# pfe-rs/lk-s-2022-estimacija-pokreta

Hardware: AMD Instinct MI355X
Metric: Mpix/s flow (1024x436, bcd_times=4) (higher is better)
Workload: dtype f64; 1 GPU; single 1024x436 Sintel-shape pair per step per GPU, forward only, bcd_times=4 (BASELINE.json configs[1]); cells 64x27, 150 labels/px; pairs_in_flight_per_gpu=7, mode=batch

## Files before the change

lk-s-2022-estimacija-pokreta_amd/csrc/bcd.hip:

```cpp
#include "dflow_common.h"

#define BCD_THREADS 192
#ifndef BCD_MINWAVES
#define BCD_MINWAVES 5
#endif
#define BCD_MASK_WORDS 5
#define BCD_BLK 5
#define BCD_LIST 15
#define BCD_LDS_LABELS 256
#define BCD_TB_STEPS 32
#define BCD_GROUPS 3
#define BCD_CAP_B01 40
#define BCD_CAP_B2 16
#define BCD_CAP_C01 24
#define BCD_CAP_C2 8
#define BCD_ROW_B (2 * BCD_CAP_B01 + BCD_CAP_B2)
#define BCD_ROW_C (2 * BCD_CAP_C01 + BCD_CAP_C2)
#define BCD_ROW_BC (BCD_ROW_B + BCD_ROW_C + 2)
#define BCD_POOL_DIV 32

#define BLK_MORE 0x800u
#define BLK_HAS_B 0x8000u
#define BLK_HAS_C 0x80000u
#define BLK_EMPTY_X 0xFFFFFFFFu
#define BLK_EMPTY_Y 0x000000FFu

__device__ static inline void chain_geom(int phase, int chain, int H, int W, int &ty, int &tx, int &ys, int &xs, int &len)
{
    if (phase == 0) { ty = 0; tx = 2 * chain; ys = 1; xs = 0; len = H; }
    else if (phase == 1) { ty = 2 * chain; tx = W - 1; ys = 0; xs = -1; len = W; }
    else if (phase == 2) { ty = H - 1; tx = (W / 2) * 2 - 1 - 2 * chain; ys = -1; xs = 0; len = H; }
    else { ty = (H / 2) * 2 - 1 - 2 * chain; tx = 0; ys = 0; xs = 1; len = W; }
}

struct BcdPlanes {
    uint8_t *back;
    uint2 *lab;
    uint2 *blkA;
    uint2 *blkBC;
    uint32_t *masks;
    uint32_t *cursor;
    uint32_t pool_rows;
};

#ifndef BCD_RANGE_BYTES
#define BCD_RANGE_BYTES 768
#endif
#define BCD_RANGE_R (BCD_RANGE_BYTES - 1)
#ifndef BCD_RANGE_PITCH
#define BCD_RANGE_PITCH 5
#endif
#define BCD_RANGE_ENTRIES (DFLOW_MAX_LABELS + 1)
#ifndef BCD_LISTS_WAVE_LDS
#define BCD_LISTS_WAVE_LDS 4096
#endif
static_assert(BCD_RANGE_BYTES % 256 == 0 && BCD_RANGE_BYTES >= 256 && BCD_RANGE_BYTES <= 1024, "rank table: 1..4 dwords per lane");
static_assert(BCD_RANGE_BYTES + BCD_RANGE_ENTRIES * BCD_RANGE_PITCH * 4 <= BCD_LISTS_WAVE_LDS && BCD_LISTS_WAVE_LDS >= 1024, "a wave's LDS");
static_assert(BCD_RANGE_PITCH >= BCD_MASK_WORDS && BCD_RANGE_PITCH <= 8, "prefix-set entry pitch");

__device__ static inline void wave_lds_sync()
{
    __builtin_amdgcn_fence(__ATOMIC_RELEASE, "wavefront");
    __builtin_amdgcn_wave_barrier();
    __builtin_amdgcn_fence(__ATOMIC_ACQUIRE, "wavefront");
}
template <int CTRL, int ROWS = 0xF> __device__ static inline uint32_t dpp_or0(uint32_t v)
{
    return (uint32_t)__builtin_amdgcn_update_dpp(0, (int)v, CTRL, ROWS, 0xF, false);
}
__device__ static inline uint32_t wave_scan_add(uint32_t x)
{
    x += dpp_or0<0x111>(x); x += dpp_or0<0x112>(x); x += dpp_or0<0x114>(x); x += dpp_or0<0x118>(x);
    x += dpp_or0<0x142, 0xA>(x); x += dpp_or0<0x143, 0xC>(x);
    return x;
}
template <int CTRL, int ROWS = 0xF> __device__ static inline void sets_or_step(uint32_t (&x)[BCD_MASK_WORDS])
{
#pragma unroll
    for (int w = 0; w < BCD_MASK_WORDS; w++) x[w] |= dpp_or0<CTRL, ROWS>(x[w]);
}
__device__ static inline void wave_scan_or(uint32_t (&x)[BCD_MASK_WORDS])
{
    sets_or_step<0x111>(x); sets_or_step<0x112>(x); sets_or_step<0x114>(x); sets_or_step<0x118>(x);
    sets_or_step<0x142, 0xA>(x); sets_or_step<0x143, 0xC>(x);
}
template <int CTRL, int ROWS = 0xF> __device__ static inline int dpp_min(int v)
{
    return min(v, __builtin_amdgcn_update_dpp(v, v, CTRL, ROWS, 0xF, false));
}
__device__ static inline int wave_min(int x)
{
    x = dpp_min<0x111>(x); x = dpp_min<0x112>(x); x = dpp_min<0x114>(x); x = dpp_min<0x118>(x);
    x = dpp_min<0x142, 0xA>(x); x = dpp_min<0x143, 0xC>(x);
    return __builtin_amdgcn_readlane(x, 63);
}
__device__ static inline void sets_load(const uint32_t *e, uint32_t (&w)[BCD_MASK_WORDS])
{
    if constexpr (BCD_RANGE_PITCH % 4 == 0) {
        const uint4 a = *reinterpret_cast<const uint4 *>(e);
        w[0] = a.x; w[1] = a.y; w[2] = a.z; w[3] = a.w;
    } else if constexpr (BCD_RANGE_PITCH % 2 == 0) {
        const uint2 a = *reinterpret_cast<const uint2 *>(e), b = *reinterpret_cast<const uint2 *>(e + 2);
        w[0] = a.x; w[1] = a.y; w[2] = b.x; w[3] = b.y;
    } else {
        w[0] = e[0]; w[1] = e[1]; w[2] = e[2]; w[3] = e[3];
    }
    w[4] = e[4];
}
__device__ static inline void sets_store(uint32_t *e, const uint32_t (&w)[BCD_MASK_WORDS])
{
    if constexpr (BCD_RANGE_PITCH % 4 == 0) {
        *reinterpret_cast<uint4 *>(e) = make_uint4(w[0], w[1], w[2], w[3]);
    } else if constexpr (BCD_RANGE_PITCH % 2 == 0) {
        *reinterpret_cast<uint2 *>(e) = make_uint2(w[0], w[1]); *reinterpret_cast<uint2 *>(e + 2) = make_uint2(w[2], w[3]);
    } else {
        e[0] = w[0]; e[1] = w[1]; e[2] = w[2]; e[3] = w[3];
    }
    e[4] = w[4];
}
template <int AX> __device__ static inline int range_coord(uint32_t f)
{
    const int lo = (int)(f & 0xFFFFu), hi = (int)(f >> 16);
    return AX ? lo - hi + 65535 : lo + hi;
}

#ifndef BCD_LISTS_WAVES
#define BCD_LISTS_WAVES 8
#endif
__global__ void __launch_bounds__(256, BCD_LISTS_WAVES) bcd_lists_kernel(int H, int W, int LP, int tpsi, const uint32_t *__restrict__ proposals,
                                                        const float *__restrict__ lcosts, const int32_t *__restrict__ nprop,
                                                        BcdPlanes pl)
{
    __shared__ uint32_t s_cols[4][256];
    __shared__ __attribute__((aligned(16))) uint8_t s_wave[4][BCD_LISTS_WAVE_LDS];
    const int lane = threadIdx.x & 63, wv = threadIdx.x >> 6;
    const int q = (int)blockIdx.x * 4 + __builtin_amdgcn_readfirstlane(wv);
    if (q >= H * W) return;
    const int y = q / W, x = q % W;
    const int py = (x & 1) ? y + 1 : y - 1, sy = (x & 1) ? y - 1 : y + 1;
    const int px = (y & 1) ? x - 1 : x + 1, sx = (y & 1) ? x + 1 : x - 1;
    const bool start0 = py < 0 || py >= H, start1 = px < 0 || px >= W;
    const bool v0 = sy >= 0 && sy < H, v1 = sx >= 0 && sx < W;
    const int p0 = v0 ? sy * W + x : q, p1 = v1 ? y * W + sx : q;
    const int pn = nprop[q], tn0 = v0 ? nprop[p0] : 0, tn1 = v1 ? nprop[p1] : 0;
    const int half = lane >> 5;
    uint32_t fq[3], f[5];
#pragma unroll
    for (int j = 0; j < 3; j++) {
        const int k = lane + 64 * j;
        fq[j] = k < pn ? flow_bias(proposals[(size_t)q * LP + k]) : 0u;
        s_cols[wv][k] = fq[j];
    }
    s_cols[wv][192 + lane] = 0u;
#pragma unroll
    for (int j = 0; j < 2; j++) {
        const int k = lane + 64 * j;
        f[j] = k < tn0 ? flow_bias(proposals[(size_t)p0 * LP + k]) : 0u;
        f[2 + j] = k < tn1 ? flow_bias(proposals[(size_t)p1 * LP + k]) : 0u;
    }
    {
        const int k = 128 + (lane & 31);
        f[4] = k < (half ? tn1 : tn0) ? flow_bias(proposals[(size_t)(half ? p1 : p0) * LP + k]) : 0u;
    }
#pragma unroll
    for (int j = 0; j < 3; j++) {
        const int k = lane + 64 * j;
        if (k < LP) pl.lab[(size_t)q * LP + k] = make_uint2(fq[j], __float_as_uint(k < pn ? lcosts[(size_t)q * LP + k] : DFLOW_FILL_COST));
    }
    if (start0 || start1) {
#pragma unroll
        for (int j = 0; j < 3; j++) {
            const int k = lane + 64 * j;
            if (k < LP) {
                if (start0) pl.blkA[((size_t)q * 2 + 0) * LP + k] = make_uint2(BLK_EMPTY_X, BLK_EMPTY_Y);
                if (start1) pl.blkA[((size_t)q * 2 + 1) * LP + k] = make_uint2(BLK_EMPTY_X, BLK_EMPTY_Y);
            }
        }
    }
    if (!v0 && !v1) return;
    const uint32_t kbias = 0x80000000u - (uint32_t)tpsi;
    const uint32_t *__restrict__ colp = proposals + (size_t)q * LP;
    uint32_t m[5][BCD_MASK_WORDS];
    const bool fifth = LP > 128 && (tn0 > 128 || tn1 > 128);
    auto build = [&](auto with5) {
#pragma unroll
        for (int j = 0; j < BCD_MASK_WORDS; j++) {
#pragma unroll
            for (int g = 0; g < 5; g++) m[g][j] = 0xFFFFFFFFu;
            if (32 * j < pn) {
                const int nv = pn - 32 * j;
                auto cols8 = [&](auto hic) {
#pragma unroll
                    for (int cc = decltype(hic)::value; cc > decltype(hic)::value - 8; cc--) {
                        const uint32_t col = flow_bias(colp[32 * j + cc]);
#pragma unroll
                        for (int g = 0; g < 4; g++) m[g][j] = __builtin_amdgcn_alignbit(m[g][j], __builtin_amdgcn_sad_u16(col, f[g], kbias), 31);
                        if (decltype(with5)::value) m[4][j] = __builtin_amdgcn_alignbit(m[4][j], __builtin_amdgcn_sad_u16(col, f[4], kbias), 31);
                    }
                };
                if (nv > 24) cols8(IntC<31>());
                if (nv > 16) cols8(IntC<23>());
                if (nv > 8) cols8(IntC<15>());
                cols8(IntC<7>());
                if (nv < 32 && (nv & 7) != 0) {
                    const uint32_t inval = ~0u << nv;
#pragma unroll
                    for (int g = 0; g < 5; g++) m[g][j] |= inval;
                }
            }
        }
    };
    const int pt = min(pn, DFLOW_MAX_LABELS);
    int cq[2][3], org[2];
    bool wide = false;
#pragma unroll
    for (int j = 0; j < 3; j++) { cq[0][j] = range_coord<0>(fq[j]); cq[1][j] = range_coord<1>(fq[j]); }
#pragma unroll
    for (int ax = 0; ax < 2; ax++) {
        int mn = 1 << 18;
#pragma unroll
        for (int j = 0; j < 3; j++) if (lane + 64 * j < pt) mn = min(mn, cq[ax][j]);
        org[ax] = wave_min(mn);
#pragma unroll
        for (int j = 0; j < 3; j++) { cq[ax][j] -= org[ax]; wide |= lane + 64 * j < pt && cq[ax][j] >= BCD_RANGE_R; }
    }
    if (__ballot(wide)) {
        if (fifth) build(IntC<1>()); else build(IntC<0>());
    } else {
        constexpr int NW = BCD_RANGE_BYTES / 256;
        uint32_t *const cw = reinterpret_cast<uint32_t *>(&s_wave[wv][0]);
        const uint8_t *const cb = &s_wave[wv][0];
        uint32_t *const sets = reinterpret_cast<uint32_t *>(&s_wave[wv][BCD_RANGE_BYTES]);
        auto axis = [&](auto axc) {
            constexpr int AX = decltype(axc)::value;
#pragma unroll
            for (int i = 0; i < NW; i++) cw[lane * NW + i] = 0u;
            wave_lds_sync();
            uint32_t ord[3];
#pragma unroll
            for (int j = 0; j < 3; j++) {
                ord[j] = 0u;
                if (lane + 64 * j < pt) {
                    const uint32_t rel = (uint32_t)cq[AX][j], sh = 8u * (rel & 3u);
                    ord[j] = (atomicAdd(&cw[rel >> 2], 1u << sh) >> sh) & 0xFFu;
                }
            }
            wave_lds_sync();
            uint32_t t[NW], before[NW], tot = 0u;
#pragma unroll
            for (int i = 0; i < NW; i++) {
                t[i] = cw[lane * NW + i];
                t[i] += t[i] << 8; t[i] += t[i] << 16;
                before[i] = tot; tot += t[i] >> 24;
            }
            const uint32_t lower = wave_scan_add(tot) - tot;
#pragma unroll
            for (int i = 0; i < NW; i++) {
                const uint32_t base = lower + before[i];
                cw[lane * NW + i] = (t[i] << 8) + __builtin_amdgcn_perm(base, base, 0x00000000u);
            }
            if (lane == 0) {
                const uint32_t none[BCD_MASK_WORDS] = {0u, 0u, 0u, 0u, 0u};
                sets_store(sets, none);
            }
            wave_lds_sync();
#pragma unroll
            for (int j = 0; j < 3; j++) {
                if (lane + 64 * j < pt) {
                    const uint32_t r = (uint32_t)cb[cq[AX][j]] + ord[j], bit = 1u << (lane & 31);
                    uint32_t one[BCD_MASK_WORDS] = {0u, 0u, 0u, 0u, 0u};
                    one[2 * j] = half ? 0u : bit;
                    if (j < 2) one[2 * j + 1] = half ? bit : 0u;
                    sets_store(sets + (r + 1u) * BCD_RANGE_PITCH, one);
                }
            }
            wave_lds_sync();
            uint32_t a[3][BCD_MASK_WORDS];
#pragma unroll
            for (int i = 0; i < 3; i++) {
#pragma unroll
                for (int w = 0; w < BCD_MASK_WORDS; w++) a[i][w] = 0u;
                if (3 * lane + i <= pt) sets_load(sets + (3 * lane + i) * BCD_RANGE_PITCH, a[i]);
            }
#pragma unroll
            for (int w = 0; w < BCD_MASK_WORDS; w++) { a[1][w] |= a[0][w]; a[2][w] |= a[1][w]; }
            wave_scan_or(a[2]);
#pragma unroll
            for (int w = 0; w < BCD_MASK_WORDS; w++) {
                const uint32_t lower_lanes = dpp_or0<0x138>(a[2][w]);
                a[0][w] |= lower_lanes; a[1][w] |= lower_lanes;
            }
#pragma unroll
            for (int i = 0; i < 3; i++)
                if (3 * lane + i <= pt) sets_store(sets + (3 * lane + i) * BCD_RANGE_PITCH, a[i]);
            wave_lds_sync();
#pragma unroll
            for (int g = 0; g < 5; g++) {
                if (g < 4 || fifth) {
                    const int c = range_coord<AX>(f[g]) - org[AX];
                    const int hi = min(max(c + tpsi, 0), BCD_RANGE_R), lo = min(max(c - tpsi + 1, 0), BCD_RANGE_R);
                    uint32_t in[BCD_MASK_WORDS], out[BCD_MASK_WORDS];
                    sets_load(sets + (uint32_t)cb[hi] * BCD_RANGE_PITCH, in);
                    sets_load(sets + (uint32_t)cb[lo] * BCD_RANGE_PITCH, out);
#pragma unroll
                    for (int w = 0; w < BCD_MASK_WORDS; w++) {
                        if (AX == 0) m[g][w] = in[w] & ~out[w];
                        else m[g][w] = ~(m[g][w] & in[w] & ~out[w]);
                        asm("" : "+v"(m[g][w]));
                    }
                } else {
#pragma unroll
                    for (int w = 0; w < BCD_MASK_WORDS; w++) m[g][w] = 0xFFFFFFFFu;
                }
                if (g & 1) __builtin_amdgcn_sched_barrier(0);
            }
            wave_lds_sync();
        };
        axis(IntC<0>());
        axis(IntC<1>());
    }

    auto emit = [&](auto mergedc, const uint32_t (&mg)[BCD_MASK_WORDS], const uint32_t me, const int ig, const int tl, const int tn,
                    const bool valid, const size_t pd) {
        constexpr bool MERGED = decltype(mergedc)::value != 0;
        uint32_t w[BCD_MASK_WORDS];
        int cnt = 0;
        uint32_t dead = valid && tl < tn ? 0u : ~0u;
        asm("" : "+v"(dead));
#pragma unroll
        for (int j = 0; j < BCD_MASK_WORDS; j++) { w[j] = __builtin_amdgcn_bitop3_b32(mg[j], dead, 0u, 0x03); cnt += __popc(w[j]); }
        uint8_t *row = &s_wave[wv][16 * lane];
        *reinterpret_cast<uint4 *>(row) = make_uint4(0xFFFFFFFFu, 0xFFFFFFFFu, 0xFFFFFFFFu, 0xFFFFFFFFu);
        const int n = min(cnt, BCD_LIST);
        const bool any = __ballot(cnt > 0) != 0ull;
        if (any) {
            uint32_t wt[BCD_MASK_WORDS];
#pragma unroll
            for (int j = 0; j < BCD_MASK_WORDS; j++) wt[j] = w[j];
            if (__ballot(cnt > BCD_LIST)) {
                int extra = cnt - BCD_LIST;
#pragma unroll
                for (int j = BCD_MASK_WORDS - 1; j >= 0; j--)
                    while (extra > 0 && wt[j]) { wt[j] &= ~(0x80000000u >> __clz(wt[j])); extra--; }
            }
            uint8_t *ap = row;
#pragma unroll
            for (int j = 0; j < BCD_MASK_WORDS; j++) {
                uint32_t ww = wt[j];
                while (ww) { *ap++ = (uint8_t)(32 * j + __ffs(ww) - 1); ww &= ww - 1; }
            }
        }
        const uint4 lst = *reinterpret_cast<const uint4 *>(row);
        const uint32_t l0 = lst.x, l1 = lst.y, l2 = lst.z, l3 = lst.w;
        uint32_t c0 = 0u, c1 = 0u;
        if (any) {
            auto slots = [&](auto lo, auto hi) {
#pragma unroll
                for (int e = decltype(lo)::value; e < decltype(hi)::value; e++) {
                    const uint32_t word = e < 4 ? l0 : (e < 8 ? l1 : (e < 12 ? l2 : l3));
                    const uint32_t k = (word >> (8 * (e & 3))) & 0xFFu;
                    const uint32_t psi = flow_l1_biased(me, s_cols[wv][k]);
                    if (e < 8) c0 |= psi << (4 * e); else c1 |= psi << (4 * (e - 8));
                }
            };
            slots(IntC<0>(), IntC<BCD_BLK>());
            if (__ballot(n > BCD_BLK)) {
                slots(IntC<BCD_BLK>(), IntC<2 * BCD_BLK>());
                if (__ballot(n > 2 * BCD_BLK)) slots(IntC<2 * BCD_BLK>(), IntC<BCD_LIST>());
            }
        }
        const unsigned long long pp = (((unsigned long long)c1 << 32) | c0) & ~(~0ull << (4 * n));
        const unsigned long long hasB = __ballot(cnt > BCD_BLK), hasC = __ballot(cnt > 2 * BCD_BLK);
        uint32_t rankB = __builtin_amdgcn_mbcnt_hi((uint32_t)(hasB >> 32), __builtin_amdgcn_mbcnt_lo((uint32_t)hasB, 0u));
        uint32_t rankC = __builtin_amdgcn_mbcnt_hi((uint32_t)(hasC >> 32), __builtin_amdgcn_mbcnt_lo((uint32_t)hasC, 0u));
        if (MERGED && half) { rankB -= (uint32_t)__popc((uint32_t)hasB); rankC -= (uint32_t)__popc((uint32_t)hasC); }
        const uint32_t capB = ig < 2 ? BCD_CAP_B01 : BCD_CAP_B2, capC = ig < 2 ? BCD_CAP_C01 : BCD_CAP_C2;
        const bool storeB = cnt > BCD_BLK && rankB < capB, storeC = cnt > 2 * BCD_BLK && storeB && rankC < capC;
        const bool more = cnt > BCD_LIST || (cnt > BCD_BLK && !storeB) || (cnt > 2 * BCD_BLK && !storeC);
        const uint32_t ax = l0;
        const uint32_t ay = (l1 & 0xFFu) | (((uint32_t)pp & 0xFFFFFu) << 8) | (more ? BLK_MORE : 0u) | (storeB ? BLK_HAS_B : 0u) |
                            (storeC ? BLK_HAS_C : 0u) | ((uint32_t)(more ? 15 : min(cnt, 15)) << 28);
        const uint32_t bx = __builtin_amdgcn_alignbit(l2, l1, 8);
        const uint32_t by = ((l2 >> 8) & 0xFFu) | (((uint32_t)(pp >> 20) & 0xFFFFFu) << 8);
        const uint32_t cx = __builtin_amdgcn_alignbit(l3, l2, 16);
        const uint32_t cy = ((l3 >> 16) & 0xFFu) | (((uint32_t)(pp >> 40) & 0xFFFFFu) << 8);
        if (valid && tl < LP) pl.blkA[pd * (size_t)LP + tl] = make_uint2(ax, ay);
        if (storeB) pl.blkBC[pd * BCD_ROW_BC + ig * BCD_CAP_B01 + rankB] = make_uint2(bx, by);
        if (storeC) pl.blkBC[pd * BCD_ROW_BC + BCD_ROW_B + ig * BCD_CAP_C01 + rankC] = make_uint2(cx, cy);
        const unsigned long long dense = __ballot(more);
        if (dense) {
            uint32_t base = 0u;
            if (lane == 0) base = atomicAdd(pl.cursor, (uint32_t)__popcll(dense));
            base = (uint32_t)__builtin_amdgcn_readfirstlane((int)base);
            uint32_t rank = __builtin_amdgcn_mbcnt_hi((uint32_t)(dense >> 32), __builtin_amdgcn_mbcnt_lo((uint32_t)dense, 0u));
            if (MERGED) {
                const uint32_t nlo = (uint32_t)__popc((uint32_t)dense);
                if ((lane & 31) == 0 && (half ? (dense >> 32) != 0ull : (uint32_t)dense != 0u))
                    reinterpret_cast<uint32_t *>(pl.blkBC + pd * BCD_ROW_BC + BCD_ROW_B + BCD_ROW_C)[ig] = base + (half ? nlo : 0u);
            } else if (lane == 0) {
                reinterpret_cast<uint32_t *>(pl.blkBC + pd * BCD_ROW_BC + BCD_ROW_B + BCD_ROW_C)[ig] = base;
            }
            const uint32_t slot = base + rank;
            if (more && slot < pl.pool_rows) {
                uint32_t *out = pl.masks + (size_t)slot * BCD_MASK_WORDS;
#pragma unroll
                for (int j = 0; j < BCD_MASK_WORDS; j++) out[j] = w[j];
            }
        }
    };
    const size_t pd0 = (size_t)p0 * 2 + 0, pd1 = (size_t)p1 * 2 + 1;
    if (v0) {
        emit(IntC<0>(), m[0], f[0], 0, lane, tn0, true, pd0);
        if (LP > 64) emit(IntC<0>(), m[1], f[1], 1, 64 + lane, tn0, true, pd0);
    }
    if (v1) {
        emit(IntC<0>(), m[2], f[2], 0, lane, tn1, true, pd1);
        if (LP > 64) emit(IntC<0>(), m[3], f[3], 1, 64 + lane, tn1, true, pd1);
    }
    if (LP > 128) emit(IntC<1>(), m[4], f[4], 2, 128 + (lane & 31), half ? tn1 : tn0, half ? v1 : v0, half ? pd1 : pd0);
}

#ifndef BCD_MAX_BATCH
#define BCD_MAX_BATCH 8
#endif
struct BcdPass {
    const int32_t *nprop;
    int32_t *bestlabels;
    BcdPlanes pl;
};
struct BcdArgs {
    int H, W, LP, tpsi, phase;
    double lamda;
    BcdPass pass[BCD_MAX_BATCH];
};

struct Cand {
    double v; int k;
};

__device__ static inline void cand_min(Cand &a, double ov, int ok)
{
    const bool take = ov < a.v || (ov == a.v && ok < a.k);
    a.v = take ? ov : a.v;
    a.k = take ? ok : a.k;
}

template <int CTRL> __device__ static inline void cand_dpp(const Cand &a, double &ov, int &ok)
{
    const int lo = __double2loint(a.v), hi = __double2hiint(a.v);
    const int olo = __builtin_amdgcn_update_dpp(lo, lo, CTRL, 0xF, 0xF, false);
    const int ohi = __builtin_amdgcn_update_dpp(hi, hi, CTRL, 0xF, 0xF, false);
    ok = __builtin_amdgcn_update_dpp(a.k, a.k, CTRL, 0xF, 0xF, false);
    ov = __hiloint2double(ohi, olo);
}

#define DPP_ROW_SHL1 0x101
#define DPP_ROW_SHL2 0x102
#define DPP_ROW_SHL4 0x104
#define DPP_ROW_SHL8 0x108

__device__ static inline void wave_min_lane0(Cand &pm)
{
    double ov; int ok;
    cand_dpp<DPP_ROW_SHL1>(pm, ov, ok); cand_min(pm, ov, ok);
    cand_dpp<DPP_ROW_SHL2>(pm, ov, ok); cand_min(pm, ov, ok);
    cand_dpp<DPP_ROW_SHL4>(pm, ov, ok); cand_min(pm, ov, ok);
    cand_dpp<DPP_ROW_SHL8>(pm, ov, ok); cand_min(pm, ov, ok);
    const int lo = __double2loint(pm.v), hi = __double2hiint(pm.v);
#pragma unroll
    for (int r = 1; r < 4; r++) {
        const double rv = __hiloint2double(__builtin_amdgcn_readlane(hi, 16 * r), __builtin_amdgcn_readlane(lo, 16 * r));
        const int rk = __builtin_amdgcn_readlane(pm.k, 16 * r);
        cand_min(pm, rv, rk);
    }
}

__device__ static inline uint32_t wave_u32_min_asm(uint32_t x)
{
    asm volatile("s_nop 1\n\t"
                 "v_min_u32_dpp %0, %0, %0 row_shl:1 row_mask:0xf bank_mask:0xf\n\t"
                 "s_nop 1\n\t"
                 "v_min_u32_dpp %0, %0, %0 row_shl:2 row_mask:0xf bank_mask:0xf\n\t"
                 "s_nop 1\n\t"
                 "v_min_u32_dpp %0, %0, %0 row_shl:4 row_mask:0xf bank_mask:0xf\n\t"
                 "s_nop 1\n\t"
                 "v_min_u32_dpp %0, %0, %0 row_shl:8 row_mask:0xf bank_mask:0xf\n\t"
                 "s_nop 0"
                 : "+v"(x));
    const uint32_t a = (uint32_t)__builtin_amdgcn_readlane((int)x, 0), b = (uint32_t)__builtin_amdgcn_readlane((int)x, 16);
    const uint32_t c = (uint32_t)__builtin_amdgcn_readlane((int)x, 32), d = (uint32_t)__builtin_amdgcn_readlane((int)x, 48);
    const uint32_t ab = a < b ? a : b, cd = c < d ? c : d;
    return ab < cd ? ab : cd;
}
__device__ static inline unsigned long long wave_key_min_asm(unsigned long long key, int *first_lane)
{
    const uint32_t hi = (uint32_t)(key >> 32), lo = (uint32_t)key;
    const uint32_t mh = wave_u32_min_asm(hi);
    const unsigned long long tie = __ballot(hi == mh);
    uint32_t ml; int fl;
    fl = __ffsll((long long)tie) - 1;
    ml = (uint32_t)__builtin_amdgcn_readlane((int)lo, fl);
    if (__builtin_expect(__popcll(tie) != 1, 0)) {
        ml = wave_u32_min_asm(hi == mh ? lo : 0xFFFFFFFFu);
        fl = __ffsll((long long)__ballot(hi == mh && lo == ml)) - 1;
    }
    *first_lane = fl;
    return ((unsigned long long)mh << 32) | ml;
}

__device__ static inline uint32_t lane_rank(unsigned long long mask)
{
    return __builtin_amdgcn_mbcnt_hi((uint32_t)(mask >> 32), __builtin_amdgcn_mbcnt_lo((uint32_t)mask, 0u));
}

#define BCD_BACK_PITCH BCD_THREADS

typedef const __attribute__((address_space(1))) char *gptr_t;
__device__ static inline gptr_t uniform_ptr(const void *p)
{
    const unsigned long long v = (unsigned long long)p;
    const uint32_t lo = __builtin_amdgcn_readfirstlane((uint32_t)v), hi = __builtin_amdgcn_readfirstlane((uint32_t)(v >> 32));
    return (gptr_t)(((unsigned long long)hi << 32) | lo);
}
__device__ static inline unsigned long long ballot64(bool b) { return __builtin_amdgcn_ballot_w64(b); }

__global__ void __launch_bounds__(BCD_THREADS, BCD_MINWAVES) bcd_chain_kernel(BcdArgs a)
{
    __shared__ double s_dp[2 * BCD_LDS_LABELS];
    __shared__ unsigned long long permv[2 * 4];
    __shared__ int permi[2 * 4 + 4];
    __shared__ __attribute__((aligned(16))) uint8_t tb[BCD_TB_STEPS * BCD_BACK_PITCH];
    extern __shared__ __attribute__((aligned(16))) uint32_t s_dyn[];
    uint32_t *bestf = s_dyn + 1;
    int *tnl;
    int *s_label = permi + 8;

    const int tid = threadIdx.x, lane = tid & 63, wave = __builtin_amdgcn_readfirstlane(tid >> 6);
    const int chain = blockIdx.x;
    const int W = a.W, LP = a.LP;
    const bool owner = tid < LP;
    const unsigned long long ownmask = ballot64(owner);
    const int tl = owner ? tid : LP - 1;
    int ty0, tx0, ys, xs, len;
    chain_geom(a.phase, chain, a.H, W, ty0, tx0, ys, xs, len);
    const int pstep = ys * W + xs;
    const int pix0 = ty0 * W + tx0;
    const int dir = ys != 0 ? 0 : 1;
    const int dirp = ys + xs;
    const uint32_t tpsi = (uint32_t)a.tpsi;
    const double tpsi_d = (double)a.tpsi;
    const double lamda = a.lamda;
    const BcdPass &ps = a.pass[blockIdx.y];
    const int32_t *g_nprop = ps.nprop;
    int32_t *g_best = ps.bestlabels;
    const uint2 *g_lab = ps.pl.lab;
    const uint32_t *g_masks = ps.pl.masks;
    const uint2 *g_bc = ps.pl.blkBC;
    const uint32_t pool_rows = ps.pl.pool_rows;
    uint8_t *back = ps.pl.back + ((size_t)chain * len) * BCD_BACK_PITCH;

    tnl = (int *)(bestf + len + 2);
    for (int i = tid; i < 2 * BCD_LDS_LABELS; i += BCD_THREADS) s_dp[i] = 1e300;
    for (int i = tid; i < len; i += BCD_THREADS) {
        int pix = pix0 + i * pstep;
        bestf[i] = g_lab[(size_t)pix * LP + g_best[pix]].x;
        tnl[i] = g_nprop[pix];
    }
    if (tid == 0) { bestf[-1] = 0u; bestf[len] = 0u; bestf[len + 1] = 0u; }
    __syncthreads();

    const uint32_t offl = (uint32_t)tl * 8u;
    const long long rowl = (long long)LP * 8, rowg = (long long)BCD_ROW_BC * 8;
    const long long strA = (long long)pstep * 2 * rowl, strL = (long long)pstep * rowl, strG = (long long)pstep * 2 * rowg;
    gptr_t pA = uniform_ptr((const char *)ps.pl.blkA + ((long long)pix0 * 2 + dir) * rowl);
    gptr_t pL = uniform_ptr((const char *)ps.pl.lab + (long long)pix0 * rowl);
    gptr_t pB = uniform_ptr((const char *)ps.pl.blkBC + ((long long)pix0 * 2 + dir) * rowg + (long long)wave * (BCD_CAP_B01 * 8));
    const uint32_t coff = (uint32_t)(BCD_ROW_B * 8 + wave * (BCD_CAP_C01 * 8) - wave * (BCD_CAP_B01 * 8));
    int nextA = 0, nextG = 0;
    auto advA = [&]() { const bool m = nextA + 1 < len; pA += m ? strA : 0; pL += m ? strL : 0; nextA++; };
    auto advG = [&]() { const bool m = nextG + 1 < len; pB += m ? strG : 0; nextG++; };
    auto ld8 = [](gptr_t base, uint32_t off) {
        const unsigned long long v = *reinterpret_cast<const __attribute__((address_space(1))) unsigned long long *>(base + off);
        return make_uint2((uint32_t)v, (uint32_t)(v >> 32));
    };
    auto fetchBC = [&](const uint2 &blkA, uint2 &B, uint2 &C) {
        const bool hb = owner && (blkA.y & BLK_HAS_B) != 0u, hc = owner && (blkA.y & BLK_HAS_C) != 0u;
        const unsigned long long mb = ballot64(hb);
        B = make_uint2(BLK_EMPTY_X, BLK_EMPTY_Y); C = make_uint2(BLK_EMPTY_X, BLK_EMPTY_Y);
        if (mb) {
            if (hb) B = ld8(pB, lane_rank(mb) * 8u);
            const unsigned long long mc = ballot64(hc);
            if (mc) { if (hc) C = ld8(pB, coff + lane_rank(mc) * 8u); }
        }
        advG();
    };
    uint2 A0, L0 = ld8(pL, offl); advA();
    uint2 A1 = ld8(pA, offl), L1 = ld8(pL, offl); advA();
    uint2 A2 = ld8(pA, offl), L2 = ld8(pL, offl); advA();
    uint2 A3 = ld8(pA, offl), L3 = ld8(pL, offl); advA();
    uint2 B1, C1, B0, C0;
    advG();
    fetchBC(A1, B1, C1);
    fetchBC(A2, B0, C0);

    {
        const uint32_t Fc = L0.x;
        const int ip = dirp, im = -dirp;
        const uint32_t s1 = (ip >= 0 && ip < len) ? min(tpsi, flow_l1_biased(Fc, bestf[ip])) : 0u;
        const uint32_t s2 = (im >= 0 && im < len) ? min(tpsi, flow_l1_biased(Fc, bestf[im])) : 0u;
        unsigned long long key = ~0ull;
        if (owner && tl < tnl[0]) {
            const double d0 = __dadd_rn((double)(s1 + s2), __dmul_rn(lamda, (double)__uint_as_float(L0.y)));
            s_dp[tl] = d0;
            key = (unsigned long long)__double_as_longlong(__dadd_rn(tpsi_d, d0));
        }
        int fl;
        const unsigned long long m = wave_key_min_asm(key, &fl);
        if (lane == 0) { permv[wave] = m; permi[wave] = wave * 64 + fl; }
    }
    A0 = ld8(pA, offl); L0 = ld8(pL, offl); advA();
    __syncthreads();

    int pn = tnl[0];
    __attribute__((address_space(1))) uint8_t *backrow = (__attribute__((address_space(1))) uint8_t *)uniform_ptr(back + BCD_BACK_PITCH);
    int tn_nx = tnl[1];
    uint32_t bfp_nx = bestf[1 + dirp], bfm_nx = bestf[1 - dirp];
    auto step = [&](auto curc, auto edgec, const int i, uint2 &inA, uint2 &inL, uint2 &inB, uint2 &inC, const uint2 &nxA) __attribute__((always_inline)) {
        constexpr int CUR = decltype(curc)::value;
        constexpr bool EDGE = decltype(edgec)::value != 0;
        const char *prev = reinterpret_cast<const char *>(s_dp + (CUR ^ 1) * BCD_LDS_LABELS);
        const int tn = tn_nx;
        const uint32_t bfp = bfp_nx, bfm = bfm_nx;
        tn_nx = tnl[min(i + 1, len - 1)];
        bfp_nx = bestf[i + 1 + dirp]; bfm_nx = bestf[i + 1 - dirp];
        const uint32_t ax = inA.x, ay = inA.y, bx = inB.x, by = inB.y, cx = inC.x, cy = inC.y;
        const uint32_t Fc = inL.x;
        const float lc = __uint_as_float(inL.y);
        const unsigned long long actmask = ballot64(tl < tn) & ownmask;
        const bool act = owner && tl < tn;
        uint32_t ad[BCD_BLK]; double dd[BCD_BLK];
#pragma unroll
        for (int j = 0; j < BCD_BLK; j++) {
            ad[j] = ((j < 4 ? ax >> (8 * j) : ay) & 0xFFu) << 3;
            dd[j] = *reinterpret_cast<const double *>(prev + ad[j]);
        }
        asm volatile("" ::: "memory");
        inA = ld8(pA, offl); inL = ld8(pL, offl); advA();
        fetchBC(nxA, inB, inC);
        Cand perm;
        double small;
        {
            const unsigned long long p0 = permv[(CUR ^ 1) * 4], p1 = permv[(CUR ^ 1) * 4 + 1], p2 = permv[(CUR ^ 1) * 4 + 2];
            const int i0 = permi[(CUR ^ 1) * 4], i1 = permi[(CUR ^ 1) * 4 + 1], i2 = permi[(CUR ^ 1) * 4 + 2];
            uint32_t lim1 = tpsi, lim2 = tpsi;
            if (EDGE) {
                const int ip = i + dirp, im = i - dirp;
                lim1 = (ip >= 0 && ip < len) ? tpsi : 0u; lim2 = (im >= 0 && im < len) ? tpsi : 0u;
            }
            const uint32_t s1 = min(flow_l1_biased(Fc, bfp), lim1);
            const uint32_t s2 = min(flow_l1_biased(Fc, bfm), lim2);
            unsigned long long pmn = p0; int pix_ = i0;
            if (p1 < pmn) { pmn = p1; pix_ = i1; }
            if (p2 < pmn) { pmn = p2; pix_ = i2; }
            perm.v = __longlong_as_double((long long)pmn); perm.k = pix_;
            small = __dadd_rn(__dadd_rn(__dmul_rn(lamda, (double)lc), (double)s1), (double)s2);
        }
        auto node = [](double &va, uint32_t &ka, const double vb, const uint32_t kb) {
            const bool t = vb < va;
            va = __builtin_fmin(va, vb); ka = t ? kb : ka;
        };
        auto block_min = [&](double (&d)[BCD_BLK], uint32_t (&k)[BCD_BLK], const uint32_t y, double &v, uint32_t &kk) {
#pragma unroll
            for (int j = 0; j < BCD_BLK; j++) d[j] = __dadd_rn(d[j], (double)((y >> (8 + 4 * j)) & 7u));
            node(d[0], k[0], d[1], k[1]); node(d[2], k[2], d[3], k[3]);
            node(d[0], k[0], d[2], k[2]); node(d[0], k[0], d[4], k[4]);
            v = d[0]; kk = k[0];
        };
        double bestv; uint32_t besta;
        block_min(dd, ad, ay, bestv, besta);
        if ((ballot64((ay >> 28) > BCD_BLK) & actmask) != 0ull) {
            uint32_t a2[BCD_BLK]; double d2[BCD_BLK];
#pragma unroll
            for (int j = 0; j < BCD_BLK; j++) { a2[j] = ((j < 4 ? bx >> (8 * j) : by) & 0xFFu) << 3; d2[j] = *reinterpret_cast<const double *>(prev + a2[j]); }
            { double vb; uint32_t kb; block_min(d2, a2, by, vb, kb); node(bestv, besta, vb, kb); }
            if (__builtin_expect((ballot64((ay >> 28) > 2 * BCD_BLK) & actmask) != 0ull, 0)) {
#pragma unroll
                for (int j = 0; j < BCD_BLK; j++) { a2[j] = ((j < 4 ? cx >> (8 * j) : cy) & 0xFFu) << 3; d2[j] = *reinterpret_cast<const double *>(prev + a2[j]); }
                { double vc; uint32_t kc; block_min(d2, a2, cy, vc, kc); node(bestv, besta, vc, kc); }
                const bool more = act && (ay & BLK_MORE) != 0u;
                const unsigned long long moremask = ballot64(more);
                if (__builtin_expect(moremask != 0ull, 0)) {
                    const int klast = (int)(((ay & BLK_HAS_C) ? cy : (ay & BLK_HAS_B) ? by : ay) & 0xFFu);
                    const size_t cpix = (size_t)(pix0 + i * pstep), ppix = (size_t)(pix0 + (i - 1) * pstep);
                    const uint2 *plab = g_lab + ppix * LP;
                    unsigned long long w0 = 0, w1 = 0, w2 = 0;
                    if (more) {
                        const uint32_t mbase = reinterpret_cast<const uint32_t *>(g_bc + (cpix * 2 + dir) * BCD_ROW_BC + BCD_ROW_B + BCD_ROW_C)[wave];
                        const uint32_t slot = mbase + lane_rank(moremask);
                        if (slot < pool_rows) {
                            const uint32_t *mrow = g_masks + (size_t)slot * BCD_MASK_WORDS;
                            w0 = (unsigned long long)mrow[0] | ((unsigned long long)mrow[1] << 32);
                            w1 = (unsigned long long)mrow[2] | ((unsigned long long)mrow[3] << 32);
                            w2 = (unsigned long long)mrow[4];
                        } else {
                            for (int k = klast + 1; k < pn; k++) {
                                const unsigned long long bit = flow_l1_biased(Fc, plab[k].x) < tpsi ? 1ull << (k & 63) : 0ull;
                                if (k < 64) w0 |= bit; else if (k < 128) w1 |= bit; else w2 |= bit;
                            }
                        }
                        const int b = klast & 63;
                        const unsigned long long keep = b == 63 ? 0ull : (~0ull << (b + 1));
                        if (klast < 64) w0 &= keep; else if (klast < 128) { w0 = 0; w1 &= keep; } else { w0 = 0; w1 = 0; w2 &= keep; }
                    }
                    int base = 0;
                    auto next_bit = [&](bool &valid) {
                        if (w0 == 0) { w0 = w1; w1 = w2; w2 = 0; base += 64; if (w0 == 0) { w0 = w1; w1 = 0; base += 64; } }
                        valid = w0 != 0;
                        int k = 0;
                        if (valid) { k = base + __ffsll((long long)w0) - 1; w0 &= w0 - 1; }
                        return k;
                    };
                    while (w0 | w1 | w2) {
                        bool v[4]; int kk[4]; double d4[4]; uint32_t ff[4];
#pragma unroll
                        for (int j = 0; j < 4; j++) kk[j] = next_bit(v[j]);
#pragma unroll
                        for (int j = 0; j < 4; j++) { d4[j] = *reinterpret_cast<const double *>(prev + 8 * kk[j]); ff[j] = plab[kk[j]].x; }
#pragma unroll
                        for (int j = 0; j < 4; j++) {
                            const double c = __dadd_rn(d4[j], (double)flow_l1_biased(Fc, ff[j]));
                            const bool t = v[j] && c < bestv;
                            bestv = t ? c : bestv; besta = t ? (uint32_t)kk[j] << 3 : besta;
                        }
                    }
                }
            }
        }
        unsigned long long key;
        {
            const bool found = bestv < 1e300;
            const double mincost = found ? bestv : perm.v;
            const int pl_ = found ? (int)(besta >> 3) : perm.k;
            const double dpc = __dadd_rn(mincost, small);
            s_dp[CUR * BCD_LDS_LABELS + tid] = dpc;
            backrow[tid] = (uint8_t)pl_;
            backrow += BCD_BACK_PITCH;
            key = act ? (unsigned long long)__double_as_longlong(__dadd_rn(tpsi_d, dpc)) : ~0ull;
        }
        {
            int fl;
            const unsigned long long m = wave_key_min_asm(key, &fl);
            if (lane == 0) { permv[CUR * 4 + wave] = m; permi[CUR * 4 + wave] = wave * 64 + fl; }
        }
        asm volatile("s_waitcnt lgkmcnt(0)" ::: "memory");
        __builtin_amdgcn_s_barrier();
        asm volatile("" ::: "memory");
        pn = tn;
    };
    int i = 1;
    for (; i + 4 < len; i += 4) {
        step(IntC<1>(), IntC<0>(), i, A1, L1, B1, C1, A3);
        step(IntC<0>(), IntC<0>(), i + 1, A2, L2, B0, C0, A0);
        step(IntC<1>(), IntC<0>(), i + 2, A3, L3, B1, C1, A1);
        step(IntC<0>(), IntC<0>(), i + 3, A0, L0, B0, C0, A2);
    }
    if (i < len) step(IntC<1>(), IntC<1>(), i, A1, L1, B1, C1, A3);
    if (i + 1 < len) step(IntC<0>(), IntC<1>(), i + 1, A2, L2, B0, C0, A0);
    if (i + 2 < len) step(IntC<1>(), IntC<1>(), i + 2, A3, L3, B1, C1, A1);
    if (i + 3 < len) step(IntC<0>(), IntC<1>(), i + 3, A0, L0, B0, C0, A2);
    const int cur = (len & 1) ? 1 : 0;

    if (tid < 64) {
        const double *dp = s_dp + (cur ^ 1) * BCD_LDS_LABELS;
        Cand m; m.v = 800000.0; m.k = 0x7fffffff;
        for (int k = lane; k < pn; k += 64) { double c = dp[k]; if (c < m.v) { m.v = c; m.k = k; } }
        wave_min_lane0(m);
        if (tid == 0) *s_label = m.k == 0x7fffffff ? 0 : m.k;
    }
    __syncthreads();
    int plb = *s_label;
    if (tid == 0) g_best[pix0 + (len - 1) * pstep] = plb;
    for (int hi = len - 1; hi >= 1; hi -= BCD_TB_STEPS) {
        const int lo = max(1, hi - BCD_TB_STEPS + 1);
        const int nbytes = (hi - lo + 1) * BCD_BACK_PITCH;
        const uint4 *src = reinterpret_cast<const uint4 *>(back + (size_t)lo * BCD_BACK_PITCH);
        for (int j = tid; j < nbytes / 16; j += BCD_THREADS) reinterpret_cast<uint4 *>(tb)[j] = src[j];
        __syncthreads();
        if (tid == 0) {
            for (int i2 = hi; i2 >= lo; i2--) {
                plb = tb[(i2 - lo) * BCD_BACK_PITCH + plb];
                g_best[pix0 + (i2 - 1) * pstep] = plb;
            }
            *s_label = plb;
        }
        __syncthreads();
        plb = *s_label;
    }
}

static void phase_dims(const dflow_params *p, int phase, int &nchains, int &len)
{
    int H = p->pich, W = p->picw;
    if (phase == 0) { nchains = (W + 1) / 2; len = H; }
    else if (phase == 1) { nchains = (H + 1) / 2; len = W; }
    else if (phase == 2) { nchains = W / 2; len = H; }
    else { nchains = H / 2; len = W; }
}

static uint32_t pool_rows_of(const dflow_params *p)
{
    const size_t rows = (size_t)p->pich * p->picw * 2 * p->label_pitch / BCD_POOL_DIV;
    return (uint32_t)(rows < 4096 ? 4096 : rows);
}

static BcdPlanes planes_of(const dflow_params *p, void *ws, size_t *bytes = nullptr)
{
    const size_t n = (size_t)p->pich * p->picw;
    size_t back = 0;
    for (int ph = 0; ph < 4; ph++) {
        int nchains, len;
        phase_dims(p, ph, nchains, len);
        const size_t b = (size_t)nchains * len * BCD_BACK_PITCH;
        if (b > back) back = b;
    }
    WsCarver c(ws);
    BcdPlanes pl;
    pl.pool_rows = pool_rows_of(p);
    pl.back = c.take<uint8_t>(back);
    pl.lab = c.take<uint2>(n * p->label_pitch);
    pl.blkA = c.take<uint2>(n * 2 * p->label_pitch);
    pl.blkBC = c.take<uint2>(n * 2 * BCD_ROW_BC);
    pl.masks = c.take<uint32_t>((size_t)pl.pool_rows * BCD_MASK_WORDS);
    pl.cursor = c.take<uint32_t>(256 / sizeof(uint32_t));
    if (bytes) *bytes = c.bytes;
    return pl;
}

size_t bcd_ws_bytes(const dflow_params *p) { size_t b; planes_of(p, nullptr, &b); return b; }

int launch_bcd_prepare(const dflow_params *p, const uint32_t *proposals, const float *lcosts, const int32_t *nprop, void *ws,
                       hipStream_t s)
{
    long long items = (long long)p->pich * p->picw;
    DFLOW_HIP(hipMemsetAsync(planes_of(p, ws).cursor, 0, 256, s));
    hipLaunchKernelGGL(bcd_lists_kernel, dim3((unsigned)((items + 3) / 4)), dim3(256), 0, s, p->pich, p->picw, p->label_pitch,
                       p->tpsi, proposals, lcosts, nprop, planes_of(p, ws));
    return dflow_check_launch("bcd_lists_kernel");
}

int launch_bcd_phase_batch(const dflow_params *p, int npass, const int32_t *const *nprop, int32_t *const *bestlabels, int phase,
                           void *const *ws, hipStream_t s)
{
    int nchains, len;
    phase_dims(p, phase, nchains, len);
    if (nchains == 0) return DFLOW_OK;
    size_t shmem = (size_t)(len + 4) * sizeof(uint32_t) + (size_t)len * sizeof(int);
    for (int b0 = 0; b0 < npass; b0 += BCD_MAX_BATCH) {
        const int nb = npass - b0 < BCD_MAX_BATCH ? npass - b0 : BCD_MAX_BATCH;
        BcdArgs a;
        a.H = p->pich; a.W = p->picw; a.LP = p->label_pitch; a.tpsi = p->tpsi; a.phase = phase; a.lamda = p->lamda;
        for (int b = 0; b < BCD_MAX_BATCH; b++) {
            const int src = b0 + (b < nb ? b : 0);
            a.pass[b].nprop = nprop[src]; a.pass[b].bestlabels = bestlabels[src]; a.pass[b].pl = planes_of(p, ws[src]);
        }
        hipLaunchKernelGGL(bcd_chain_kernel, dim3(nchains, nb), dim3(BCD_THREADS), shmem, s, a);
        int rc = dflow_check_launch("bcd_chain_kernel");
        if (rc) return rc;
    }
    return DFLOW_OK;
}

int launch_bcd_phase(const dflow_params *p, const int32_t *nprop, int32_t *bestlabels, int phase, void *ws, hipStream_t s)
{
    void *wsv = ws;
    return launch_bcd_phase_batch(p, 1, &nprop, &bestlabels, phase, &wsv, s);
}
```

Measured before the change: 42.76 Mpix/s.

## Run backtrack in a single wave using register-resident double-buffered traceback rows

The traceback after the chain DP no longer stages backpointer rows through LDS with block-wide barriers and a serial thread-0 walk. Instead only wave 0 continues: each lane loads one dword of 32 rows into registers, and the walk uses readlane for the serial dependency and writelane to gather the outputs. Loads for the next 32-step chunk are issued while the current chunk is walked, and the other waves exit early. This removes the LDS tb array, which may help occupancy, and it removes the barriers. The cost is more VGPRs (two 32-entry register arrays) and an explicit vmcnt wait.

```diff
diff --git a/lk-s-2022-estimacija-pokreta_amd/csrc/bcd.hip b/lk-s-2022-estimacija-pokreta_amd/csrc/bcd.hip
--- a/lk-s-2022-estimacija-pokreta_amd/csrc/bcd.hip
+++ b/lk-s-2022-estimacija-pokreta_amd/csrc/bcd.hip
@@ -529,7 +529,6 @@
     __shared__ double s_dp[2 * BCD_LDS_LABELS];
     __shared__ unsigned long long permv[2 * 4];
     __shared__ int permi[2 * 4 + 4];
-    __shared__ __attribute__((aligned(16))) uint8_t tb[BCD_TB_STEPS * BCD_BACK_PITCH];
     extern __shared__ __attribute__((aligned(16))) uint32_t s_dyn[];
     uint32_t *bestf = s_dyn + 1;
     int *tnl;
@@ -770,6 +769,7 @@
     if (i + 3 < len) step(IntC<0>(), IntC<1>(), i + 3, A0, L0, B0, C0, A2);
     const int cur = (len & 1) ? 1 : 0;
 
+    asm volatile("s_waitcnt vmcnt(0)" ::: "memory");
     if (tid < 64) {
         const double *dp = s_dp + (cur ^ 1) * BCD_LDS_LABELS;
         Cand m; m.v = 800000.0; m.k = 0x7fffffff;
@@ -778,23 +778,50 @@
         if (tid == 0) *s_label = m.k == 0x7fffffff ? 0 : m.k;
     }
     __syncthreads();
-    int plb = *s_label;
+    if (wave != 0) return;
+    int plb = __builtin_amdgcn_readfirstlane(*s_label);
     if (tid == 0) g_best[pix0 + (len - 1) * pstep] = plb;
-    for (int hi = len - 1; hi >= 1; hi -= BCD_TB_STEPS) {
-        const int lo = max(1, hi - BCD_TB_STEPS + 1);
-        const int nbytes = (hi - lo + 1) * BCD_BACK_PITCH;
-        const uint4 *src = reinterpret_cast<const uint4 *>(back + (size_t)lo * BCD_BACK_PITCH);
-        for (int j = tid; j < nbytes / 16; j += BCD_THREADS) reinterpret_cast<uint4 *>(tb)[j] = src[j];
-        __syncthreads();
-        if (tid == 0) {
-            for (int i2 = hi; i2 >= lo; i2--) {
-                plb = tb[(i2 - lo) * BCD_BACK_PITCH + plb];
-                g_best[pix0 + (i2 - 1) * pstep] = plb;
-            }
-            *s_label = plb;
-        }
-        __syncthreads();
-        plb = *s_label;
+    const gptr_t brow = uniform_ptr(back);
+    const uint32_t boff = (uint32_t)(lane < 48 ? lane : 47) * 4u;
+    auto tb_load_first = [&](uint32_t (&R)[BCD_TB_STEPS], const int hi) __attribute__((always_inline)) {
+#pragma unroll
+        for (int j = 0; j < BCD_TB_STEPS; j++)
+            R[j] = *reinterpret_cast<const __attribute__((address_space(1))) uint32_t *>(brow + (uint32_t)(max(hi - j, 0) * BCD_BACK_PITCH) + boff);
+    };
+    auto tb_load = [&](uint32_t (&R)[BCD_TB_STEPS], const int hi) __attribute__((always_inline)) {
+        const gptr_t top = brow + (uint32_t)(hi * BCD_BACK_PITCH);
+#pragma unroll
+        for (int j = 0; j < BCD_TB_STEPS; j++)
+            R[j] = *reinterpret_cast<const __attribute__((address_space(1))) uint32_t *>(top + boff - j * BCD_BACK_PITCH);
+    };
+    auto tb_walk = [&](const uint32_t (&R)[BCD_TB_STEPS], const int hi, const int cnt) __attribute__((always_inline)) {
+        int outv = 0;
+#pragma unroll
+        for (int j = 0; j < BCD_TB_STEPS; j++) {
+            if (j < cnt) {
+                const uint32_t w = (uint32_t)__builtin_amdgcn_readlane((int)R[j], plb >> 2);
+                plb = (int)((w >> ((plb & 3) * 8)) & 0xFFu);
+                asm volatile("v_writelane_b32 %0, %1, %2" : "+v"(outv) : "s"(plb), "n"(j));
+            }
+        }
+        if (lane < cnt) g_best[pix0 + (hi - 1 - lane) * pstep] = outv;
+    };
+    int hi = len - 1;
+    if (hi < 1) return;
+    uint32_t RA[BCD_TB_STEPS], RB[BCD_TB_STEPS];
+    const int cnt0 = ((hi - 1) & (BCD_TB_STEPS - 1)) + 1;
+    tb_load_first(RA, hi);
+    if (hi > cnt0) tb_load(RB, hi - cnt0);
+    tb_walk(RA, hi, cnt0);
+    hi -= cnt0;
+    while (hi >= 1) {
+        if (hi > BCD_TB_STEPS) tb_load(RA, hi - BCD_TB_STEPS);
+        tb_walk(RB, hi, BCD_TB_STEPS);
+        hi -= BCD_TB_STEPS;
+        if (hi < 1) break;
+        if (hi > BCD_TB_STEPS) tb_load(RB, hi - BCD_TB_STEPS);
+        tb_walk(RA, hi, BCD_TB_STEPS);
+        hi -= BCD_TB_STEPS;
     }
 }
 
```

Measured after the change: 42.65 Mpix/s. Within noise of the previous version (-0.3%).
